# VisionLearningGroup/UDA_PoseEstimation

Hardware: AMD Instinct MI355X
Metric: images/sec (student+teacher step) 256x256 b=32 (higher is better)
Workload: dtype bf16

## Files before the change

### uda_poseestimation_amd/csrc/conv_plan.h

```cpp
#pragma once
#include <atomic>
#include <mutex>
#include <vector>
#include "igemm.h"

struct Policy : udapose_policy {
    Policy() : udapose_policy{} {
        igemm_tile = -1; igemm_h3 = 1; igemm_lean = 1; igemm_short_lds = 1; igemm_tap0 = 1;
        wgrad_tile = -1; wgrad_ksplit = -1; wgrad_fastgeo = 2;
        wgrad_group = 1; wgrad_stages = 128; wgrad_group_stem = 1;
        bn_bwd_fused = 1; bn_fwd_chunked = 1; bn_bwd_chunked = 1; bn_bwd_pre_legacy = 0;
        igemm_wg_min = 512; wgrad_row3 = 1; bn3_mask = 1; stem_fused = 1; debug_sync = 0;
        igemm_big_min = 0; patch_conv = 2; eval_fold = 1; bn_xcd_rows = 1; wgrad_det = 1; igemm_ns3_k = 0;
        timeline = nullptr; wgrad_order = 1; wgrad_fastgeo_strided = 1;
    }
};
inline const Policy& default_policy() { static const Policy p; return p; }

template <auto Kernel>
inline void max_dynamic_lds(int bytes) {
    static std::atomic<unsigned long long> done{0};
    static std::mutex mu;
    int dev = 0;
    (void)hipGetDevice(&dev);
    const unsigned long long bit = 1ull << (dev & 63);
    if (done.load(std::memory_order_acquire) & bit) return;
    std::lock_guard<std::mutex> lk(mu);
    if (done.load(std::memory_order_relaxed) & bit) return;
    (void)hipFuncSetAttribute((const void*)Kernel, hipFuncAttributeMaxDynamicSharedMemorySize, bytes);
    done.fetch_or(bit, std::memory_order_release);
}

struct ConvGeom {
    int N, Hi, Wi, Ci;
    int Co, KH, KW, stride, pad;
    int transposed;
    int reflect;
    int upsample;
    const Policy* pol = nullptr;
    const Policy& policy() const { return pol ? *pol : default_policy(); }
    int Ho() const { return transposed ? (Hi - 1) * stride - 2 * pad + KH : (((Hi << upsample) + 2 * pad - KH) / stride + 1); }
    int Wo() const { return transposed ? (Wi - 1) * stride - 2 * pad + KW : (((Wi << upsample) + 2 * pad - KW) / stride + 1); }
    bool smallc() const { return Ci == 8; }
    int KWp() const { return smallc() ? ((KW + 7) & ~7) : KW; }
    int wtaps() const { return KH * KWp(); }
};

struct TapPlan {
    std::vector<IgTap> taps;
    int nclass = 1;
    IgClass cls[4];
    const IgTap* d_taps = nullptr;
};

const TapPlan* get_tap_plan(const ConvGeom& g, int direction, hipStream_t stream = nullptr);
int conv_prepare(const ConvGeom& g);

int igemm_pick_tile(int M, int Co, int nclass, int K, int h3_ok, const Policy& pol);
int conv_h3_ok(const ConvGeom& g);
int igemm_stat_rows(int M, int Co, int nclass, int tile);
int igemm_launch(IgParams& p, int tile, hipStream_t stream, const Policy& pol);
int wgrad_pick_tile(int Rdim, int Cdim, int smallc, const Policy& pol);
int wgrad_launch(WgParams& p, int tile, int accumulate, hipStream_t stream, const Policy& pol);
// ... 43 lines not shown
```

### uda_poseestimation_amd/csrc/igemm.h

```cpp
#pragma once
#include "common.h"

struct IgTap { int dy, dx, widx, cls; };
struct IgClass { int tap_off, ntaps, oa, ob; };

#define IG_FLAG_REFLECT 1
#define IG_FLAG_UPSAMPLE 2
#define IG_FLAG_RELU 4
#define IG_FLAG_OUT_F32 8
#define IG_FLAG_F32 128
#define IG_FLAG_SPLIT 64
#define IG_FLAG_MIRROR 2048
#define IG_FLAG_TAP0 1024
#define IG_FLAG_BSMASK 32
#define IG_FLAG_SMALLC 16

struct IgParams {
    const elem_t* x;
    const elem_t* w;
    void* y;
    const elem_t* res;
    const float* bias;
    const float* scale;
    float* stats;
    const IgTap* taps;
    int N, Hi, Wi, Ci;
    int Ho, Wo, Co;
    int Hg, Wg;
    int s, os;
    int M;
    int wtaps;
    int flags;
    int nclass;
    IgClass cls[4];
    FastDiv div_hw, div_w;
    int m_tiles, n_tiles;
    int tap0;
    unsigned long long* dbg;
    const elem_t* bs_y;
    const elem_t* bs_z;
    const float* bs_mean;
    const float* bs_invstd;
    const float* bs_gamma;
    const float* bs_beta;
};

struct WgParams {
    const elem_t* dy;
    const elem_t* x;
    float* dw;
    const IgTap* taps;
    int N, Hi, Wi, Ci;
    int Ho, Wo, Co;
    int Hg, Wg;
    int s, os;
    int M;
    int wtaps;
    int flags;
    int nclass;
    IgClass cls[4];
    FastDiv div_hw, div_w;
    int ksplit;
    int msteps_per_split;
    int r_tiles, c_tiles;
    int total_taps;
    int rows_valid;
    int kw;
    unsigned part_stride;
};
struct WgGroupBlk { int prob, local; };
#define WG_FLAG_SWAP 32
#define WG_FLAG_DW_WS 256
#define WG_FLAG_FASTGEO 512
#define WG_FLAG_FAST2 16384
#define WG_FLAG_FASTGEO_S 32768
#define WG_FLAG_ROW3_OK 8192
#define WG_FLAG_ROW3 4096
#define WG_FLAG_ATOMIC 64
```

### uda_poseestimation_amd/csrc/net.hip

```cpp
#include <algorithm>
#include <deque>
#include <functional>
#include <queue>
#include <cstdio>
#include <cstdlib>
#include <string>
#include <type_traits>
#include <vector>
#include "net.h"
#include "pointwise.h"
#include "optim.h"

namespace {

inline size_t align_up(size_t v, size_t a = 256) { return (v + a - 1) / a * a; }
static thread_local int t_dbg_sync = 0;
struct DbgSyncScope { int prev; explicit DbgSyncScope(int on) : prev(t_dbg_sync) { t_dbg_sync = on; } ~DbgSyncScope() { t_dbg_sync = prev; } };
#define CK(expr) do { int _e = (expr); \
    if (t_dbg_sync) { fprintf(stderr, "[udapose] net.hip:%d %s\n", __LINE__, #expr); fflush(stderr); \
        if (hipDeviceSynchronize() != hipSuccess) { fprintf(stderr, "[udapose] FAILED at net.hip:%d\n", __LINE__); return UDAPOSE_ERR_LAUNCH; } } \
    if (_e != UDAPOSE_OK) return _e; } while (0)

struct ConvL {
    ConvGeom g;
// ... 31 lines not shown
    DevTable& operator=(DevTable&& o) noexcept { if (this != &o) { reset(); d = o.d; n = o.n; o.d = nullptr; o.n = 0; } return *this; }
    ~DevTable() { reset(); }
    void reset() { if (d) (void)hipFree(d); d = nullptr; n = 0; }
    int upload(const std::vector<T>& v) {
        reset();
        if (hipMalloc((void**)&d, v.size() * sizeof(T)) != hipSuccess) { d = nullptr; return UDAPOSE_ERR_LAUNCH; }
        if (hipMemcpy(d, v.data(), v.size() * sizeof(T), hipMemcpyHostToDevice) != hipSuccess) { reset(); return UDAPOSE_ERR_LAUNCH; }
        n = v.size();
        return UDAPOSE_OK;
    }
};
template <class J> struct JobTab {
    DevTable<J> jobs; DevTable<int> blk_job, blk_sub;
    int nblocks() const { return (int)blk_job.n; }
    void reset() { jobs.reset(); blk_job.reset(); blk_sub.reset(); }
    int upload(const std::vector<J>& j, const std::vector<int>& bj, const std::vector<int>& bs) {
        if (jobs.upload(j) == UDAPOSE_OK && blk_job.upload(bj) == UDAPOSE_OK && blk_sub.upload(bs) == UDAPOSE_OK) return UDAPOSE_OK;
        reset();
        return UDAPOSE_ERR_LAUNCH;
    }
};
struct PackJobH { const float* src; elem_t* dst; int A, T, B, kind; long long n; };

struct Net {
    int layers[4], K, N, H, W;
    int split_dz_idx = -1;
    Policy policy;
    int f32 = 0;
    int strict = 0;
    int fwd_only = 0;
    struct Scratch { size_t need[6] = {0, 0, 0, 0, 0, 0}, off[6] = {0, 0, 0, 0, 0, 0}; bool sizing = false; } sc;
    int deconv_bias = 0;
    size_t es = 2;
    int n_params = 0, n_buffers = 0;
    std::vector<long long> param_numel;
    ConvL stem; BnL stem_bn;
    size_t x8_off = 0, pool_off = 0, poolidx_off = 0;
    size_t fx8_off = 0, fpool_off = 0;
    int Hs = 0, Ws = 0, Hp = 0, Wp = 0;
    std::vector<Block> blocks;
    ConvL up[3]; BnL up_bn[3];
    ConvL head;
    size_t head_out_off = 0;
    int fc_w_idx = -1, fc_b_idx = -1;
    size_t act_bytes = 0, wpack_bytes = 0, ws_bytes = 0;
    size_t ws_slab = 0, ws_slabf = 0, ws_coef = 0, ws_gbuf[6] = {0, 0, 0, 0, 0, 0}, ws_dyhead = 0, ws_dwtmp = 0, ws_headbwd = 0;
    size_t ws_wgpart = 0, ws_wgpart_bytes = 0;
    size_t gbuf_bytes = 0;
    int Hout = 0, Wout = 0;
    struct PackTab : JobTab<PackJobH> { const void* key0 = nullptr; const void* key1 = nullptr; const void* keyw = nullptr; };
    PackTab pack_fwd, pack_all;
    struct WgGroup {
        float k_beta = -1.f; int k_stages = 0; int k_part = 0;
        bool k_det = false, k_stem = false; int k_order = 0, k_geo_s = 0;
        size_t part_bytes = 0;
        std::vector<std::pair<int, ptrdiff_t>> rel;
        std::vector<size_t> rel_bytes;
        std::vector<int> rel_cls;
        DevTable<WgParams> d_tab[WG_CLASSES]; DevTable<WgGroupBlk> d_blk[WG_CLASSES]; int per_xcd[WG_CLASSES] = {};
        double flops[WG_CLASSES] = {};
        std::vector<std::pair<ptrdiff_t, size_t>> zero;
        DevTable<ZeroJob> d_zero;
        DevTable<SumJob> d_sum; DevTable<int> d_sum_blk; int n_sum_blk = 0;
        int n_sum_ws_blk = 0;
        std::vector<SumJob> h_sum;
        unsigned long long last_use = 0;
    };
    std::deque<WgGroup> wg_groups;
    struct UpdTab : JobTab<TailJob> {
                    const void* k_ps = nullptr; const void* k_pt = nullptr; const void* k_g = nullptr; const void* k_m = nullptr;
                    const void* k_ws = nullptr; const void* k_wt = nullptr;
                    int kind = 0, ngroups = 1; };
    UpdTab upd;
    struct Deferred { const WgGroup* G = nullptr; char* wsA = nullptr; char* wsB = nullptr; char* gA = nullptr; char* gB = nullptr; } deferred;
    const WgGroup* upd_sum_group = nullptr;
    DevTable<BnRunJob> d_runjobs; const void* runjobs_key = nullptr;
    unsigned long long wg_tick = 0;
};

template <class F, class... A> int walk_rc(F& fn, A&... a) {
    if constexpr (std::is_void_v<decltype(fn(a...))>) { fn(a...); return UDAPOSE_OK; }
    else return fn(a...);
}
template <class N, class F> int for_each_layer(N& n, F fn) {
    int rc = walk_rc(fn, n.stem, n.stem_bn);
    for (size_t i = 0; rc == UDAPOSE_OK && i < n.blocks.size(); ++i) {
        auto& b = n.blocks[i];
        if ((rc = walk_rc(fn, b.c1, b.b1)) == UDAPOSE_OK && (rc = walk_rc(fn, b.c2, b.b2)) == UDAPOSE_OK && (rc = walk_rc(fn, b.c3, b.b3)) == UDAPOSE_OK && b.has_ds)
            rc = walk_rc(fn, b.cd, b.bd);
    }
    for (int i = 0; rc == UDAPOSE_OK && i < 3; ++i) rc = walk_rc(fn, n.up[i], n.up_bn[i]);
    return rc;
}
template <class N, class F> int for_each_conv(N& n, F fn) { return for_each_layer(n, [&](auto& c, auto&) { return walk_rc(fn, c); }); }
template <class N, class F> int for_each_bn(N& n, F fn) { return for_each_layer(n, [&](auto&, auto& b) { return walk_rc(fn, b); }); }

size_t act_alloc(Net& n, size_t bytes) { size_t o = n.act_bytes; n.act_bytes = align_up(o + bytes); return o; }
size_t wp_alloc(Net& n, size_t bytes) { size_t o = n.wpack_bytes; n.wpack_bytes = align_up(o + bytes); return o; }

enum { SC_Y = 0, SC_A, SC_B, SC_MID, SC_MID2, SC_DS, SC_COUNT };
size_t sc_take(Net& n, int slot, size_t bytes) {
    if (n.sc.sizing) { n.sc.need[slot] = std::max(n.sc.need[slot], align_up(bytes)); return 0; }
    return n.sc.off[slot];
}
void add_conv(Net& n, ConvL& c, int Hi, int Wi, int Ci, int Co, int K, int stride, int pad, int transposed, size_t in_off, size_t fin_off, bool need_bwd_pack,
              int y_slot = -1) {
    c.g = ConvGeom{n.N, Hi, Wi, Ci, Co, K, K, stride, pad, transposed, 0, 0};
// ... 382 lines not shown
    }
    if (c.g.smallc() && grouped_wgrad && n.policy.wgrad_group_stem) {
    } else if (c.g.smallc()) {
        float* tmp = (float*)(ws + n.ws_dwtmp);
        CK(conv_wgrad(s, c.g, dy, xin, tmp, 0, -1));
        CK(pw_unpack_strided(s, tmp, (float*)grads[c.w_idx], c.g.Co, c.g.KH, c.g.KWp(), c.g.KW, 8, 3, (long)c.g.KH * c.g.KW * 3, (long)c.g.KW * 3, 3, 1,
                             beta));
    } else if (!grouped_wgrad) {
        CK(conv_wgrad(s, c.g, dy, xin, (float*)grads[c.w_idx], beta != 0.f, -1));
    }
    if (need_dx) {
        elem_t* dx = pool.get();
        if (!dx) return UDAPOSE_ERR_ARG;
        CK(conv_dgrad(s, c.g, dy, (const elem_t*)(wpack + c.wb_off), dx, dx_res, dx_f32, next));
        *dx_out = dx;
    }
    return UDAPOSE_OK;
}

DgradBnStat bn_stat_of(const Net& n, const ConvL& c, const BnL& b, const void* const* params, char* act, char* ws, int relu) {
    DgradBnStat st;
    const float* save = (const float*)(act + b.save_off);
    st.y = (const elem_t*)(act + c.y_off);
    st.z = relu == 1 ? (const elem_t*)(act + b.z_off) : nullptr;
    st.mask = (relu == 1 && b.mask_off && n.policy.bn3_mask) ? (const unsigned char*)(act + b.mask_off) : nullptr;
    st.mean = save; st.invstd = save + b.C;
    st.gamma = (const float*)params[b.g_idx]; st.beta = (const float*)params[b.b_idx];
    st.slab = (float*)(ws + n.ws_slabf);
    return st;
}


inline int split_block(const Net& n) { return n.layers[0] + n.layers[1]; }

struct PartSel { bool head_up; int hi, lo; bool stem; };
PartSel part_sel(const Net& n, int part) {
    const int nb = (int)n.blocks.size(), split = split_block(n);
    if (part == 1) return PartSel{true, nb - 1, split, false};
    if (part == 2) return PartSel{false, split - 1, 0, true};
    return PartSel{true, nb - 1, 0, true};
}
template <class N, class F> int for_each_conv_wgrad(N& n, const PartSel& sel, F fn) {
    int rc = UDAPOSE_OK;
    for (int i = 2; sel.head_up && rc == UDAPOSE_OK && i >= 0; --i) rc = walk_rc(fn, n.up[i]);
    for (int bi = sel.hi; rc == UDAPOSE_OK && bi >= sel.lo; --bi) {
        auto& b = n.blocks[bi];
        if ((rc = walk_rc(fn, b.c3)) == UDAPOSE_OK && (rc = walk_rc(fn, b.c2)) == UDAPOSE_OK && (!b.has_ds || (rc = walk_rc(fn, b.cd)) == UDAPOSE_OK))
            rc = walk_rc(fn, b.c1);
    }
    return rc;
}

#define WG_DEAL_RUN 32
struct WgUnit { int prob, base, nblk, st; long load; };
double wg_model_finish(const std::vector<WgUnit>& runs, const std::vector<int>& lst, int slots = 128) {
    std::priority_queue<double, std::vector<double>, std::greater<double>> free_at;
    for (int i = 0; i < slots; ++i) free_at.push(0.0);
    double end = 0.0;
    for (int ui : lst)
        for (int l = 0; l < runs[ui].nblk; ++l) {
            const double t = free_at.top() + runs[ui].st + 4;
            free_at.pop();
            free_at.push(t);
            end = std::max(end, t);
        }
    return end;
}
void wg_deal(const std::vector<WgUnit>& units, int order, std::vector<WgUnit>& runs, std::vector<int> lst[8]) {
    runs.clear();
    for (const WgUnit& u : units) {
        const int step = order == 0 ? u.nblk : WG_DEAL_RUN;
        for (int l0 = 0; l0 < u.nblk; l0 += step) {
            const int cnt = std::min(step, u.nblk - l0);
            runs.push_back(WgUnit{u.prob, u.base + l0, cnt, u.st, (long)cnt * (u.st + 4)});
        }
    }
    std::vector<int> idx(runs.size());
    for (size_t i = 0; i < idx.size(); ++i) idx[i] = (int)i;
    if (order == 0) std::stable_sort(idx.begin(), idx.end(), [&](int a, int b) { return runs[a].load > runs[b].load; });
    else std::stable_sort(idx.begin(), idx.end(), [&](int a, int b) { return runs[a].st != runs[b].st ? runs[a].st > runs[b].st : runs[a].load > runs[b].load; });
    long load[8] = {0, 0, 0, 0, 0, 0, 0, 0};
    for (int k = 0; k < 8; ++k) lst[k].clear();
    for (int ui : idx) {
        int x = 0;
        for (int k = 1; k < 8; ++k) if (load[k] < load[x]) x = k;
        load[x] += runs[ui].load;
        lst[x].push_back(ui);
    }
}

int build_wg_group(Net& n, Net::WgGroup& G, void* const* grads, float beta, int part, bool sizing = false, size_t* need = nullptr) {
    const PartSel sel = part_sel(n, part);
    const bool upper = sel.head_up, lower = sel.stem;
    std::vector<WgParams> tab[WG_CLASSES];
    std::vector<WgUnit> units[WG_CLASSES];
    G.zero.clear();
    G.rel.clear();
    G.rel_bytes.clear();
    G.rel_cls.clear();
    for (int t = 0; t < WG_CLASSES; ++t) G.flops[t] = 0.0;
    std::vector<SumJob> sums;
    size_t part_cur = 0;
    const bool det = n.policy.wgrad_det && n.policy.wgrad_group;
    auto make_partial = [&](WgParams& p, long long dst_off, int dst_ws, int Cdim) -> int {
        const int ms_total = (p.M + 63) / 64, per = (ms_total + p.ksplit - 1) / p.ksplit;
        const int ks_eff = (ms_total + per - 1) / per;
        const size_t span = (size_t)p.rows_valid * p.wtaps * Cdim;
        if (span >= (1ull << 31) || (span & 3)) return UDAPOSE_ERR_UNSUPPORTED;
        p.flags = (p.flags & ~WG_FLAG_ATOMIC) | WG_FLAG_DW_WS;
        p.dw = (float*)(n.ws_wgpart + part_cur);
        p.part_stride = (unsigned)span;
        sums.push_back(SumJob{(long long)(n.ws_wgpart + part_cur), dst_off, (unsigned)span, (unsigned)span, ks_eff, dst_ws, dst_ws ? 0.f : beta, 0});
        part_cur = align_up(part_cur + (size_t)ks_eff * span * sizeof(float));
        return UDAPOSE_OK;
    };
    auto emit = [&](int t, const WgParams& p, double fl) {
        const int prob = (int)tab[t].size();
        tab[t].push_back(p);
        G.flops[t] += fl;
        const int nblk = p.r_tiles * p.c_tiles * p.total_taps;
        const int ms_total = (p.M + 63) / 64, per = (ms_total + p.ksplit - 1) / p.ksplit;
        for (int z = 0; z < p.ksplit; ++z) {
            const int st = std::min(per, ms_total - z * per);
            if (st > 0) units[t].push_back(WgUnit{prob, z * nblk, nblk, st, (long)nblk * (st + 4)});
        }
    };
    auto add_geom = [&](const ConvGeom& g, int w_idx, size_t dy_off, size_t in_off, int rows_valid) -> int {
        if (g.smallc()) return UDAPOSE_OK;
        WgParams p;
        double fl = 0.0;
        const ptrdiff_t drel = sizing ? 0 : (const char*)grads[w_idx] - (const char*)grads[0];
        G.rel.push_back({w_idx, drel});
        CK(conv_wgrad_params(g, (const elem_t*)dy_off, (const elem_t*)in_off, (float*)drel, rows_valid, &p, &fl));
        const int t = wgrad_group_plan(p, beta != 0.f, n.policy.wgrad_stages, n.policy);
        if (t < 0) return UDAPOSE_ERR_UNSUPPORTED;
        G.rel_bytes.push_back((size_t)p.rows_valid * p.wtaps * ((p.flags & WG_FLAG_SWAP) ? p.Co : p.Ci) * sizeof(float));
        if (p.ksplit > 1) {
            const bool swap = (p.flags & WG_FLAG_SWAP) != 0;
            if (det) CK(make_partial(p, (long long)drel, 0, swap ? p.Co : p.Ci));
            else if (beta == 0.f) G.zero.push_back({drel, (size_t)p.rows_valid * p.wtaps * (swap ? p.Co : p.Ci) * sizeof(float)});
        }
        G.rel_cls.push_back(t);
        emit(t, p, fl);
        return UDAPOSE_OK;
    };
    if (upper) {
        ConvGeom hg = n.head.g;
        hg.Co = 64;
        CK(add_geom(hg, n.head.w_idx, n.ws_dyhead, n.head.in_off, n.K));
        G.flops[1] -= 2.0 * n.N * n.Hout * n.Wout * 256.0 * (64 - n.K);
    }
    if (lower && n.policy.wgrad_group_stem) {
        WgParams p;
        double fl = 0.0;
        CK(conv_wgrad_params(n.stem.g, (const elem_t*)n.stem.dy_off, (const elem_t*)n.stem.in_off, (float*)n.ws_dwtmp, -2, &p, &fl));
        p.flags |= WG_FLAG_DW_WS;
        const int t = wgrad_group_plan(p, 1, n.policy.wgrad_stages, n.policy);
        if (t != 1) return UDAPOSE_ERR_UNSUPPORTED;
        if (det) CK(make_partial(p, (long long)n.ws_dwtmp, 1, 64));
        emit(t, p, fl);
    }
    CK(for_each_conv_wgrad(n, sel, [&](const ConvL& c) { return add_geom(c.g, c.w_idx, c.dy_off, c.in_off, -1); }));
    if (sizing) { if (need) *need = part_cur; return UDAPOSE_OK; }
    if (part_cur > n.ws_wgpart_bytes) return UDAPOSE_ERR_NOT_PREPARED;
    for (int t = 0; t < WG_CLASSES; ++t) {
        G.d_tab[t].reset();
        G.d_blk[t].reset();
        G.per_xcd[t] = 0;
        if (tab[t].empty()) continue;
        std::vector<int> deal[8];
        std::vector<WgUnit> runs;
        wg_deal(units[t], n.policy.wgrad_order, runs, deal);
        std::vector<WgGroupBlk> lst[8];
        for (int x = 0; x < 8; ++x)
            for (int ui : deal[x]) {
                const WgUnit& u = runs[ui];
                for (int l = 0; l < u.nblk; ++l) lst[x].push_back(WgGroupBlk{u.prob, u.base + l});
            }
        size_t per = 0;
        for (int k = 0; k < 8; ++k) per = std::max(per, lst[k].size());
        std::vector<WgGroupBlk> flat(8 * per, WgGroupBlk{-1, 0});
        for (int k = 0; k < 8; ++k) std::copy(lst[k].begin(), lst[k].end(), flat.begin() + k * per);
        CK(G.d_tab[t].upload(tab[t]));
        CK(G.d_blk[t].upload(flat));
        G.per_xcd[t] = (int)per;
    }
    G.d_zero.reset();
    bool granular = !G.zero.empty();
    for (auto& z : G.zero) granular = granular && (z.second % 16 == 0) && ((((size_t)(const char*)grads[0]) + (size_t)z.first) % 16 == 0);
    if (granular) {
        std::vector<ZeroJob> zj;
        for (auto& z : G.zero) zj.push_back(ZeroJob{(long long)z.first, (long long)(z.second / 16)});
        CK(G.d_zero.upload(zj));
    }
    G.d_sum.reset();
    G.d_sum_blk.reset();
    G.n_sum_blk = 0; G.n_sum_ws_blk = 0;
    if (!sums.empty()) {
        std::vector<int> blk;
        for (const int ws_jobs : {0, 1})
            for (size_t j = 0; j < sums.size(); ++j) {
                if ((sums[j].dst_ws != 0) != (ws_jobs != 0)) continue;
                for (unsigned c = 0; c < (sums[j].n + UDAPOSE_SPLIT_SUM_CHUNK - 1u) / UDAPOSE_SPLIT_SUM_CHUNK; ++c) {
                    blk.push_back((int)j); blk.push_back((int)c);
                    G.n_sum_ws_blk += ws_jobs;
                }
            }
        CK(G.d_sum.upload(sums));
        CK(G.d_sum_blk.upload(blk));
        G.n_sum_blk = (int)(blk.size() / 2);
    }
    G.h_sum = sums;
    G.k_beta = beta; G.k_stages = n.policy.wgrad_stages; G.k_part = part;
    G.k_det = det; G.k_stem = n.policy.wgrad_group_stem != 0; G.part_bytes = part_cur; G.k_order = n.policy.wgrad_order; G.k_geo_s = n.policy.wgrad_fastgeo_strided;
    return UDAPOSE_OK;
}

size_t wg_partial_bytes(Net& n) {
    Net::WgGroup G;
    size_t need = 0;
    if (build_wg_group(n, G, nullptr, 0.f, 0, true, &need) != UDAPOSE_OK) return 0;
    return need;
}

Net::WgGroup* find_wg_group(Net& n, void* const* grads, float beta, int part) {
    const bool det = n.policy.wgrad_det && n.policy.wgrad_group, stem = n.policy.wgrad_group_stem != 0;
    for (auto& g : n.wg_groups) {
        if (g.k_beta != beta || g.k_stages != n.policy.wgrad_stages || g.k_part != part || g.k_det != det || g.k_stem != stem ||
            g.k_order != n.policy.wgrad_order || g.k_geo_s != n.policy.wgrad_fastgeo_strided) continue;
        if (g.k_det && g.part_bytes > n.ws_wgpart_bytes) continue;
        bool same = true;
        for (auto& r : g.rel)
            if ((const char*)grads[r.first] - (const char*)grads[0] != r.second) { same = false; break; }
        if (same) return &g;
    }
    return nullptr;
}
int bind_wg_groups(Net& n, void* const* grads) {
    for (const int part : {0, 1, 2})
        for (const float beta : {0.f, 1.f}) {
            if (find_wg_group(n, grads, beta, part)) continue;
            n.wg_groups.emplace_back();
            Net::WgGroup* G = &n.wg_groups.back();
            const int rc = build_wg_group(n, *G, grads, beta, part);
            if (rc != UDAPOSE_OK) { n.wg_groups.pop_back(); return rc; }
            G->last_use = ++n.wg_tick;
        }
    return UDAPOSE_OK;
}
int wg_before(hipStream_t s, Net& n, Net::WgGroup* G, char* ws, void* const* grads, bool with_stem) {
    G->last_use = ++n.wg_tick;
    if (G->d_zero.d) {
        CK(pw_zero_multi(s, G->d_zero.d, (int)G->d_zero.n, grads[0]));
    } else {
        for (auto& z : G->zero)
            if (pw_zero(s, (char*)grads[0] + z.first, z.second) != UDAPOSE_OK) return UDAPOSE_ERR_LAUNCH;
    }
    const ConvGeom& sg = n.stem.g;
    if (with_stem && !G->k_det && pw_zero(s, ws + n.ws_dwtmp, (size_t)sg.Co * sg.KH * 8 * 8 * sizeof(float)) != UDAPOSE_OK) return UDAPOSE_ERR_LAUNCH;
    return UDAPOSE_OK;
}
int wg_after(hipStream_t s, Net& n, Net::WgGroup* G, char* ws, void* const* grads, float beta, bool with_stem, bool sums_done = false) {
    if (G->n_sum_blk && !sums_done) CK(pw_split_sum(s, G->d_sum.d, G->d_sum_blk.d, G->n_sum_blk, ws, (char*)grads[0]));
    const ConvGeom& sg = n.stem.g;
    if (with_stem)
        CK(pw_unpack_strided(s, (const float*)(ws + n.ws_dwtmp), (float*)grads[n.stem.w_idx], sg.Co, sg.KH, sg.KWp(), sg.KW, 8, 3,
                             (long)sg.KH * sg.KW * 3, (long)sg.KW * 3, 3, 1, beta));
    return UDAPOSE_OK;
}
bool wg_overlap(const Net& n, const Net::WgGroup* GA, void* const* gradsA, const Net::WgGroup* GB, void* const* gradsB, bool with_stem) {
    auto span = [&](const Net::WgGroup* G, void* const* grads, uintptr_t& lo, uintptr_t& hi) {
        lo = UINTPTR_MAX; hi = 0;
        auto add = [&](int idx, size_t bytes) {
            const uintptr_t a = (uintptr_t)grads[idx];
            lo = std::min(lo, a); hi = std::max(hi, a + bytes);
        };
        for (size_t i = 0; i < G->rel.size(); ++i) add(G->rel[i].first, G->rel_bytes[i]);
        if (with_stem) add(n.stem.w_idx, (size_t)n.stem.g.Co * n.stem.g.KH * n.stem.g.KW * 3 * sizeof(float));
    };
// ... 377 lines not shown
```

### uda_poseestimation_amd/csrc/wgrad.hip

```cpp
#include <stdlib.h>
#include "conv_plan.h"
#include "mma_tile.h"
#include "pointwise.h"

namespace {

template <int RT, int CT, int WR, int WC>
struct WgCfg {
    static constexpr int TR = RT / WR, TC = CT / WC;
    static constexpr int MT = TR / 16, NT = TC / 16;
    static constexpr int PSTR = RT * 2 + 32, QSTR = CT * 2 + 32;
    static constexpr int P_BYTES = 32 * PSTR, Q_BYTES = 32 * QSTR;
    static constexpr int P_CH = (32 * RT / 8 + 255) / 256, Q_CH = (32 * CT / 8 + 255) / 256;
    static constexpr int LDS_BYTES = 2 * (P_BYTES + Q_BYTES);
};

template <int MT, int NT>
__device__ __forceinline__ void wg_store_tile(const f32x4 (&acc)[MT][NT], int lane, int row0, int col0, int Rdim, int rows_valid, int Cdim, int wtaps, int widx,
                                              float* dw, size_t part_off, bool atomic) {
#pragma unroll
    for (int i = 0; i < MT; ++i)
#pragma unroll
        for (int j = 0; j < NT; ++j)
#pragma unroll
// ... 559 lines not shown
        }

    for (int st = 0; st < nsteps; ++st) {
        const int buf = st % NS;
        ring.step(st, nsteps, issue_stage);
        const char* P = smem + buf * R::STAGE1;
        const char* Q = P + R::P_BYTES;
#pragma unroll
        for (int kk = 0; kk < 2; ++kk) {
            union F8 { struct { s16x4 a, b; } s; elem8 v; u32x4 w; };
            F8 af[2];
#pragma unroll
            for (int i = 0; i < 2; ++i) {
                const int col = wr * 32 + i * 16 + 4 * pp;
#pragma unroll
                for (int h = 0; h < 2; ++h) {
                    const int row = 32 * kk + 16 * h + 4 * g + qq;
                    const int off = wfrag_off<64>(row, col);
                    const s16x4 v = __builtin_amdgcn_ds_read_tr16_b64_v4i16(LDS_PTR(s16x4, P + off));
                    if (h == 0) af[i].s.a = v; else af[i].s.b = v;
                }
            }
#pragma unroll
            for (int t = 0; t < 3; ++t) {
                F8 bfr[2];
#pragma unroll
                for (int j = 0; j < 2; ++j) {
                    const int col = wc * 32 + j * 16 + 4 * pp;
#pragma unroll
                    for (int h = 0; h < 2; ++h) {
                        const int row = 32 * kk + 16 * h + 4 * g + qq + t;
                        const int off = wfrag_off<64>(row, col);
                        const s16x4 v = __builtin_amdgcn_ds_read_tr16_b64_v4i16(LDS_PTR(s16x4, Q + off));
                        if (h == 0) bfr[j].s.a = v; else bfr[j].s.b = v;
                    }
                }
#pragma unroll
                for (int i = 0; i < 2; ++i) {
                    F8 a = af[i];
                    if (t == 0) { a.w[0] &= mL[kk][0]; a.w[1] &= mL[kk][1]; a.w[2] &= mL[kk][2]; a.w[3] &= mL[kk][3]; }
                    if (t == 2) { a.w[0] &= mR[kk][0]; a.w[1] &= mR[kk][1]; a.w[2] &= mR[kk][2]; a.w[3] &= mR[kk][3]; }
#pragma unroll
                    for (int j = 0; j < 2; ++j) acc[t][i][j] = UDAPOSE_MFMA_16x16x32(a.v, bfr[j].v, acc[t][i][j]);
                }
            }
        }
    }

#pragma unroll
    for (int t = 0; t < 3; ++t)
        wg_store_tile(acc[t], lane, r0 + wr * 32, c0 + wc * 32, p.Co, p.rows_valid, p.Ci, p.wtaps, 3 * by + t, p.dw, part_off, (p.flags & WG_FLAG_ATOMIC) != 0);
}

template <int RT, int CT, int WR, int WC, int NS, int PX>
__device__ __forceinline__ void wgrad_run_body(const WgParams& p, const uint32_t bx, const uint32_t by, const uint32_t bz, char* smem,
                                               const uintptr_t x_base, const uintptr_t dy_base, const uintptr_t dw_base) {
    if constexpr (RT == 64 && CT == 64 && PX == 64) {
        if (p.flags & WG_FLAG_ROW3) { wgrad_row3_body<NS>(p, bx, by, bz, smem, x_base, dy_base, dw_base); return; }
    }
    if (p.flags & WG_FLAG_FAST2) wgrad_fast2_body<RT, CT, WR, WC, NS, PX>(p, bx, by, bz, smem, x_base, dy_base, dw_base);
    else if (p.flags & WG_FLAG_FASTGEO) wgrad_dma_body<RT, CT, WR, WC, NS, PX, 1>(p, bx, by, bz, smem, x_base, dy_base, dw_base);
    else if (p.flags & WG_FLAG_FASTGEO_S) wgrad_dma_body<RT, CT, WR, WC, NS, PX, 2>(p, bx, by, bz, smem, x_base, dy_base, dw_base);
    else wgrad_dma_body<RT, CT, WR, WC, NS, PX>(p, bx, by, bz, smem, x_base, dy_base, dw_base);
}

template <int RT, int CT, int WR, int WC, int NS>
__global__ __launch_bounds__(256) void wgrad_dma_kernel(const WgParams p) {
    extern __shared__ __attribute__((aligned(16))) char smem[];
    const uint32_t gxy = gridDim.x * gridDim.y;
    const uint32_t lin = xcd_remap(blockIdx.x + gridDim.x * (blockIdx.y + gridDim.y * blockIdx.z), gxy * gridDim.z);
    const uint32_t bz = lin / gxy, bxy = lin - bz * gxy;
    const uint32_t by = bxy / gridDim.x, bx = bxy - by * gridDim.x;
    wgrad_run_body<RT, CT, WR, WC, NS, 64>(p, bx, by, bz, smem, 0, 0, 0);
}

template <int RT, int CT, int WR, int WC, int NS, int PX>
__device__ __forceinline__ void wgrad_group_dispatch(const WgParams* __restrict__ tab, const WgGroupBlk* __restrict__ blk, const uint32_t per_xcd,
                                                     const char* x_base, const char* dy_base, char* dw_base, const WgParams* __restrict__ tab2,
                                                     const WgGroupBlk* __restrict__ blk2, const char* x_base2, const char* dy_base2, char* dw_base2,
                                                     char* smem) {
    uint32_t slot = blockIdx.x >> 3;
    if (tab2) {
        if (slot & 1u) { tab = tab2; blk = blk2; x_base = x_base2; dy_base = dy_base2; dw_base = dw_base2; }
        slot >>= 1;
    }
    const WgGroupBlk b = blk[(blockIdx.x & 7u) * per_xcd + slot];
    if (b.prob < 0) return;
    const WgParams& p = tab[b.prob];
    const uint32_t gx = (uint32_t)(p.r_tiles * p.c_tiles), gxy = gx * (uint32_t)p.total_taps;
    const uint32_t bz = (uint32_t)b.local / gxy, bxy = (uint32_t)b.local - bz * gxy;
    const uint32_t by = bxy / gx, bx = bxy - by * gx;
    wgrad_run_body<RT, CT, WR, WC, NS, PX>(p, bx, by, bz, smem, (uintptr_t)x_base, (uintptr_t)dy_base, (uintptr_t)dw_base);
}

template <int RT, int CT, int WR, int WC, int NS, int PX, bool STAMP = false>
__global__ __launch_bounds__(256) __attribute__((amdgpu_waves_per_eu(4))) void wgrad_dma_group_kernel(const WgParams* __restrict__ tab, const WgGroupBlk* __restrict__ blk,
                                                              const uint32_t per_xcd, const char* x_base, const char* dy_base, char* dw_base,
                                                              const WgParams* __restrict__ tab2, const WgGroupBlk* __restrict__ blk2,
                                                              const char* x_base2, const char* dy_base2, char* dw_base2,
                                                              unsigned long long* __restrict__ stamps) {
    extern __shared__ __attribute__((aligned(16))) char smem[];
    if constexpr (STAMP) {
        unsigned long long* const st = stamps + (size_t)blockIdx.x * 8;
        const unsigned long long t0 = __builtin_amdgcn_s_memrealtime();
        uint32_t slot = blockIdx.x >> 3, pass = 0;
        if (tab2) { pass = slot & 1u; slot >>= 1; }
        const WgGroupBlk b = (pass ? blk2 : blk)[(blockIdx.x & 7u) * per_xcd + slot];
        long long stages = 0;
        if (b.prob >= 0) {
            const WgParams& p = (pass ? tab2 : tab)[b.prob];
            const uint32_t gxy = (uint32_t)(p.r_tiles * p.c_tiles) * (uint32_t)p.total_taps;
            const int bz = (int)((uint32_t)b.local / gxy), ms_total = (p.M + 63) / 64;
            stages = ms_total - bz * p.msteps_per_split < p.msteps_per_split ? ms_total - bz * p.msteps_per_split : p.msteps_per_split;
            if (p.flags & WG_FLAG_ROW3) stages |= 1ll << 32;
            if (p.flags & IG_FLAG_SMALLC) stages |= 1ll << 33;
            if (p.flags & WG_FLAG_FASTGEO_S) stages |= 1ll << 34;
            if (p.flags & WG_FLAG_SWAP) stages |= 1ll << 35;
            if (p.s == 2) stages |= 1ll << 36;
        }
        wgrad_group_dispatch<RT, CT, WR, WC, NS, PX>(tab, blk, per_xcd, x_base, dy_base, dw_base, tab2, blk2, x_base2, dy_base2, dw_base2, smem);
        __syncthreads();
        if (threadIdx.x == 0) {
            st[0] = t0; st[1] = __builtin_amdgcn_s_memrealtime(); st[2] = blockIdx.x & 7u; st[3] = slot;
            st[4] = (unsigned long long)(long long)b.prob; st[5] = (unsigned long long)stages; st[6] = pass; st[7] = RT;
        }
    } else {
        wgrad_group_dispatch<RT, CT, WR, WC, NS, PX>(tab, blk, per_xcd, x_base, dy_base, dw_base, tab2, blk2, x_base2, dy_base2, dw_base2, smem);
    }
}

template <int RT, int CT, int WR, int WC, int NS, int PX, bool STAMP = false>
int launch_wd_group(const WgParams* d_tab, const WgGroupBlk* d_blk, int per_xcd, const void* x_base, const void* dy_base, void* dw_base,
                    hipStream_t stream, const WgParams* d_tab2 = nullptr, const WgGroupBlk* d_blk2 = nullptr, const void* x_base2 = nullptr,
                    const void* dy_base2 = nullptr, void* dw_base2 = nullptr, unsigned long long* stamps = nullptr) {
    using C = WdCfg<RT, CT, WR, WC, NS, PX>;
    constexpr int LDS = (RT == 64 && CT == 64 && PX == 64 && Row3Cfg::lds_bytes(NS) > C::LDS_BYTES) ? Row3Cfg::lds_bytes(NS) : C::LDS_BYTES;
    max_dynamic_lds<wgrad_dma_group_kernel<RT, CT, WR, WC, NS, PX, STAMP>>(LDS);
    hipLaunchKernelGGL((wgrad_dma_group_kernel<RT, CT, WR, WC, NS, PX, STAMP>), dim3(8 * per_xcd * (d_tab2 ? 2 : 1)), dim3(256), LDS, stream, d_tab, d_blk,
                       (uint32_t)per_xcd, (const char*)x_base, (const char*)dy_base, (char*)dw_base, d_tab2, d_blk2, (const char*)x_base2,
                       (const char*)dy_base2, (char*)dw_base2, stamps);
    return udapose_check_launch();
}

template <int RT, int CT, int WR, int WC, int NS>
int launch_wd(WgParams& p, hipStream_t stream) {
    using C = WdCfg<RT, CT, WR, WC, NS>;
    constexpr int LDS = (RT == 64 && CT == 64 && Row3Cfg::lds_bytes(NS) > C::LDS_BYTES) ? Row3Cfg::lds_bytes(NS) : C::LDS_BYTES;
    const bool swap = (p.flags & WG_FLAG_SWAP) != 0;
    const int Rdim = swap ? p.Ci : p.Co, Cdim = swap ? p.Co : p.Ci;
    p.r_tiles = (Rdim + RT - 1) / RT;
    p.c_tiles = (Cdim + CT - 1) / CT;
    max_dynamic_lds<wgrad_dma_kernel<RT, CT, WR, WC, NS>>(LDS);
    dim3 grid(p.r_tiles * p.c_tiles, p.total_taps, p.ksplit);
    hipLaunchKernelGGL((wgrad_dma_kernel<RT, CT, WR, WC, NS>), grid, dim3(256), LDS, stream, p);
    return udapose_check_launch();
}

template <int RT, int CT, int WR, int WC>
int launch_wg(WgParams& p, hipStream_t stream) {
    using C = WgCfg<RT, CT, WR, WC>;
    const bool swap = (p.flags & WG_FLAG_SWAP) != 0;
    const bool smallc = (p.flags & IG_FLAG_SMALLC) != 0;
    const int Rdim = swap ? p.Ci : p.Co, Cdim = swap ? p.Co : p.Ci;
    p.r_tiles = (Rdim + RT - 1) / RT;
    p.c_tiles = smallc ? 1 : (Cdim + CT - 1) / CT;
    const int tapsy = smallc ? p.total_taps / 4 : p.total_taps;
    dim3 grid(p.r_tiles * p.c_tiles, tapsy, p.ksplit);
    hipLaunchKernelGGL((wgrad_kernel<RT, CT, WR, WC>), grid, dim3(256), C::LDS_BYTES, stream, p);
    return udapose_check_launch();
}

}

static bool wg_fastgeo_ok(const WgParams& p, const Policy& pol) {
    const bool pow2 = ((p.Hi & (p.Hi - 1)) | (p.Wi & (p.Wi - 1))) == 0;
    return pol.wgrad_fastgeo && !(p.flags & (IG_FLAG_SMALLC | WG_FLAG_SWAP)) && p.s == 1 && p.os == 1 && p.nclass == 1 && p.Hg == p.Hi && p.Wg == p.Wi &&
           p.Hg == p.Ho && p.Wg == p.Wo && pow2 && p.Hi > 0 && p.M < (1 << 24) && p.Ci < (1 << 24) && p.Co < (1 << 24) &&
           (long long)p.M * (p.Ci > p.Co ? p.Ci : p.Co) < (1ll << 31);
}

static bool wg_fastgeo_strided_ok(const WgParams& p, const Policy& pol) {
    if (!pol.wgrad_fastgeo || !pol.wgrad_fastgeo_strided || wg_fastgeo_ok(p, pol)) return false;
    const int dims[6] = {p.Hg, p.Wg, p.Hi, p.Wi, p.Ho, p.Wo};
    for (int d : dims) if (d <= 0 || (d & (d - 1))) return false;
    if ((p.s != 1 && p.s != 2) || (p.os != 1 && p.os != 2) || p.Ho != p.Hg * p.os || p.Wo != p.Wg * p.os) return false;
    if (p.nclass < 1 || p.nclass > 4) return false;
    for (int c = 0; c < p.nclass; ++c)
        if (p.cls[c].oa < 0 || p.cls[c].oa >= p.os || p.cls[c].ob < 0 || p.cls[c].ob >= p.os) return false;
    if (p.flags & IG_FLAG_SMALLC) {
// ... 45 lines not shown
        p.flags |= WG_FLAG_ROW3;
        p.total_taps = 3;
    }
    const long tiles = (long)((Rdim + RT[tile] - 1) / RT[tile]) * (smallc ? 1 : (Cdim + CT[tile] - 1) / CT[tile]) *
                       (smallc ? p.total_taps / 4 : p.total_taps);
    const bool dma = !smallc && (tile == 0 || tile == 1) && (p.Ci % 64 == 0) && (p.Co % 64 == 0);
    const int ms_total = dma ? (p.M + 63) / 64 : (p.M + 31) / 32;
    int ks = wg_split_count(tiles, ms_total, tile, 1 << 30);
    if (pol.wgrad_ksplit > 0) { ks = pol.wgrad_ksplit; while (ks > 1 && ms_total / ks < 1) ks /= 2; }
    p.ksplit = ks;
    p.part_stride = 0;
    p.msteps_per_split = (ms_total + ks - 1) / ks;
    if (ks > 1 || accumulate) p.flags |= WG_FLAG_ATOMIC; else p.flags &= ~WG_FLAG_ATOMIC;
    if (ks > 1 && !accumulate) {
        const size_t n = (size_t)Rdim * p.wtaps * Cdim;
        if (pw_zero(stream, p.dw, n * sizeof(float)) != UDAPOSE_OK) return UDAPOSE_ERR_LAUNCH;
    }
    wg_classify(p, pol, dma);
    if (dma) return tile == 0 ? launch_wd<128, 128, 2, 2, 2>(p, stream) : launch_wd<64, 64, 2, 2, 4>(p, stream);
    switch (tile) {
        case 0: return launch_wg<128, 128, 2, 2>(p, stream);
        case 1: return launch_wg<64, 64, 2, 2>(p, stream);
        case 2: return launch_wg<64, 32, 2, 2>(p, stream);
        case 3: return launch_wg<32, 128, 1, 4>(p, stream);
        default: return UDAPOSE_ERR_ARG;
    }
}

int wgrad_group_plan(WgParams& p, int accumulate, int stages_per_block, const Policy& pol) {
    const bool smallc = (p.flags & IG_FLAG_SMALLC) != 0;
    const bool swap = (p.flags & WG_FLAG_SWAP) != 0;
    if (smallc && (swap || p.Co % 64 != 0 || p.kw <= 0 || p.kw > 8)) return -1;
    if (!smallc && (p.Ci % 64 != 0 || p.Co % 64 != 0)) return -1;
    const int Rdim = swap ? p.Ci : p.Co, Cdim = smallc ? 64 : (swap ? p.Co : p.Ci);
    p.div_hw = make_fastdiv((uint32_t)(p.Hg * p.Wg));
    p.div_w = make_fastdiv((uint32_t)p.Wg);
    int tile = (Rdim >= 128 && Cdim >= 128) ? 0 : 1;
    if (wg_row3_ok(p, pol)) {
        tile = 1;
        p.flags |= WG_FLAG_ROW3;
        p.total_taps = 3;
    }
    const int TRr = tile == 0 ? 128 : 64, TCc = tile == 1 ? 64 : 128;
    p.r_tiles = (Rdim + TRr - 1) / TRr;
    p.c_tiles = (Cdim + TCc - 1) / TCc;
    const int ms_total = (p.M + 63) / 64;
    int ks = (ms_total + stages_per_block / 2) / stages_per_block;
    if (ks < 1) ks = 1;
    p.ksplit = ks;
    p.part_stride = 0;
    p.msteps_per_split = (ms_total + ks - 1) / ks;
    if (ks > 1 || accumulate) p.flags |= WG_FLAG_ATOMIC; else p.flags &= ~WG_FLAG_ATOMIC;
    wg_classify(p, pol, true);
    return tile;
}

int wgrad_group_launch(hipStream_t stream, int tile, const WgParams* d_tab, const WgGroupBlk* d_blk, int per_xcd, const void* x_base,
                       const void* dy_base, void* dw_base, const WgParams* d_tab2, const WgGroupBlk* d_blk2, const void* x_base2,
                       const void* dy_base2, void* dw_base2, unsigned long long* stamps) {
    if (per_xcd <= 0) return UDAPOSE_OK;
    if (stamps) {
        if (tile == 0) return launch_wd_group<128, 128, 2, 2, 2, 32, true>(d_tab, d_blk, per_xcd, x_base, dy_base, dw_base, stream, d_tab2, d_blk2, x_base2, dy_base2, dw_base2, stamps);
        return launch_wd_group<64, 64, 2, 2, 2, 64, true>(d_tab, d_blk, per_xcd, x_base, dy_base, dw_base, stream, d_tab2, d_blk2, x_base2, dy_base2, dw_base2, stamps);
    }
    if (tile == 0) return launch_wd_group<128, 128, 2, 2, 2, 32>(d_tab, d_blk, per_xcd, x_base, dy_base, dw_base, stream, d_tab2, d_blk2, x_base2, dy_base2, dw_base2);
    return launch_wd_group<64, 64, 2, 2, 2, 64>(d_tab, d_blk, per_xcd, x_base, dy_base, dw_base, stream, d_tab2, d_blk2, x_base2, dy_base2, dw_base2);
}

int wgrad_parts_plan(int M, int Ci, int Co, int total_taps, int* tile_out) {
    const int tile = (Co >= 128 && Ci >= 128 && total_taps >= 9) ? 0 : 1;
    const int RT = tile == 0 ? 128 : 64;
    const long tiles = (long)((Co + RT - 1) / RT) * ((Ci + RT - 1) / RT) * total_taps;
    const int ms_total = (M + 63) / 64;
    const int ks = wg_split_count(tiles, ms_total, tile, 64);
    if (tile_out) *tile_out = tile;
    return ks;
}

int wgrad_launch_parts(WgParams& p, float* parts, hipStream_t stream) {
    if (p.Ci % 64 || p.Co % 64 || (p.flags & (IG_FLAG_SMALLC | WG_FLAG_SWAP | WG_FLAG_ROW3_OK))) return UDAPOSE_ERR_ARG;
    int tile = 1;
    const int ks = wgrad_parts_plan(p.M, p.Ci, p.Co, p.total_taps, &tile);
    p.div_hw = make_fastdiv((uint32_t)(p.Hg * p.Wg));
    p.div_w = make_fastdiv((uint32_t)p.Wg);
    p.ksplit = ks;
    p.msteps_per_split = ((p.M + 63) / 64 + ks - 1) / ks;
    p.dw = parts;
    p.part_stride = (unsigned)((size_t)p.Co * p.wtaps * p.Ci);
    p.flags &= ~(WG_FLAG_ATOMIC | WG_FLAG_FASTGEO | WG_FLAG_FAST2 | WG_FLAG_FASTGEO_S | WG_FLAG_ROW3);
    return tile == 0 ? launch_wd<128, 128, 2, 2, 2>(p, stream) : launch_wd<64, 64, 2, 2, 4>(p, stream);
}
```

Baseline: 2034.

## Add stem row-group wgrad path sharing dy tile across kernel rows

Adds a specialized weight-gradient body for the small-channel stem conv that processes up to three kernel rows per block. One dy tile staged in LDS is reused against several x row tiles, which cuts redundant dy loads and block count. The scheduler cost model is adjusted for the heavier per-stage work, and the policy default enables the path. The new path carries more accumulators, which adds register pressure, and each group now does more serialized work.

```diff
diff --git a/uda_poseestimation_amd/csrc/conv_plan.h b/uda_poseestimation_amd/csrc/conv_plan.h
--- a/uda_poseestimation_amd/csrc/conv_plan.h
+++ b/uda_poseestimation_amd/csrc/conv_plan.h
@@ -8,7 +8,7 @@
     Policy() : udapose_policy{} {
         igemm_tile = -1; igemm_h3 = 1; igemm_lean = 1; igemm_short_lds = 1; igemm_tap0 = 1;
         wgrad_tile = -1; wgrad_ksplit = -1; wgrad_fastgeo = 2;
-        wgrad_group = 1; wgrad_stages = 128; wgrad_group_stem = 1;
+        wgrad_group = 1; wgrad_stages = 128; wgrad_group_stem = 2;
         bn_bwd_fused = 1; bn_fwd_chunked = 1; bn_bwd_chunked = 1; bn_bwd_pre_legacy = 0;
         igemm_wg_min = 512; wgrad_row3 = 1; bn3_mask = 1; stem_fused = 1; debug_sync = 0;
         igemm_big_min = 0; patch_conv = 2; eval_fold = 1; bn_xcd_rows = 1; wgrad_det = 1; igemm_ns3_k = 0;
diff --git a/uda_poseestimation_amd/csrc/igemm.h b/uda_poseestimation_amd/csrc/igemm.h
--- a/uda_poseestimation_amd/csrc/igemm.h
+++ b/uda_poseestimation_amd/csrc/igemm.h
@@ -76,4 +76,5 @@
 #define WG_FLAG_FASTGEO_S 32768
 #define WG_FLAG_ROW3_OK 8192
 #define WG_FLAG_ROW3 4096
+#define WG_FLAG_STEMROWS 65536
 #define WG_FLAG_ATOMIC 64
diff --git a/uda_poseestimation_amd/csrc/net.hip b/uda_poseestimation_amd/csrc/net.hip
--- a/uda_poseestimation_amd/csrc/net.hip
+++ b/uda_poseestimation_amd/csrc/net.hip
@@ -107,7 +107,7 @@
     PackTab pack_fwd, pack_all;
     struct WgGroup {
         float k_beta = -1.f; int k_stages = 0; int k_part = 0;
-        bool k_det = false, k_stem = false; int k_order = 0, k_geo_s = 0;
+        bool k_det = false; int k_stem = 0, k_order = 0, k_geo_s = 0;
         size_t part_bytes = 0;
         std::vector<std::pair<int, ptrdiff_t>> rel;
         std::vector<size_t> rel_bytes;
@@ -596,6 +596,7 @@
 }
 
 #define WG_DEAL_RUN 32
+#define WG_STEMROWS_STAGE_W 5
 struct WgUnit { int prob, base, nblk, st; long load; };
 double wg_model_finish(const std::vector<WgUnit>& runs, const std::vector<int>& lst, int slots = 128) {
     std::priority_queue<double, std::vector<double>, std::greater<double>> free_at;
@@ -665,8 +666,10 @@
         const int nblk = p.r_tiles * p.c_tiles * p.total_taps;
         const int ms_total = (p.M + 63) / 64, per = (ms_total + p.ksplit - 1) / p.ksplit;
         for (int z = 0; z < p.ksplit; ++z) {
-            const int st = std::min(per, ms_total - z * per);
-            if (st > 0) units[t].push_back(WgUnit{prob, z * nblk, nblk, st, (long)nblk * (st + 4)});
+            int st = std::min(per, ms_total - z * per);
+            if (st <= 0) continue;
+            if (p.flags & WG_FLAG_STEMROWS) st = (st * WG_STEMROWS_STAGE_W + 3) / 4;
+            units[t].push_back(WgUnit{prob, z * nblk, nblk, st, (long)nblk * (st + 4)});
         }
     };
     auto add_geom = [&](const ConvGeom& g, int w_idx, size_t dy_off, size_t in_off, int rows_valid) -> int {
@@ -756,7 +759,7 @@
     }
     G.h_sum = sums;
     G.k_beta = beta; G.k_stages = n.policy.wgrad_stages; G.k_part = part;
-    G.k_det = det; G.k_stem = n.policy.wgrad_group_stem != 0; G.part_bytes = part_cur; G.k_order = n.policy.wgrad_order; G.k_geo_s = n.policy.wgrad_fastgeo_strided;
+    G.k_det = det; G.k_stem = n.policy.wgrad_group_stem; G.part_bytes = part_cur; G.k_order = n.policy.wgrad_order; G.k_geo_s = n.policy.wgrad_fastgeo_strided;
     return UDAPOSE_OK;
 }
 
@@ -768,7 +771,8 @@
 }
 
 Net::WgGroup* find_wg_group(Net& n, void* const* grads, float beta, int part) {
-    const bool det = n.policy.wgrad_det && n.policy.wgrad_group, stem = n.policy.wgrad_group_stem != 0;
+    const bool det = n.policy.wgrad_det && n.policy.wgrad_group;
+    const int stem = n.policy.wgrad_group_stem;
     for (auto& g : n.wg_groups) {
         if (g.k_beta != beta || g.k_stages != n.policy.wgrad_stages || g.k_part != part || g.k_det != det || g.k_stem != stem ||
             g.k_order != n.policy.wgrad_order || g.k_geo_s != n.policy.wgrad_fastgeo_strided) continue;
diff --git a/uda_poseestimation_amd/csrc/wgrad.hip b/uda_poseestimation_amd/csrc/wgrad.hip
--- a/uda_poseestimation_amd/csrc/wgrad.hip
+++ b/uda_poseestimation_amd/csrc/wgrad.hip
@@ -635,11 +635,121 @@
         wg_store_tile(acc[t], lane, r0 + wr * 32, c0 + wc * 32, p.Co, p.rows_valid, p.Ci, p.wtaps, 3 * by + t, p.dw, part_off, (p.flags & WG_FLAG_ATOMIC) != 0);
 }
 
+struct StemRowsCfg {
+    static constexpr int RMAX = 3, PX = 32, TILE = PX * 128, STAGE1 = (1 + RMAX) * TILE;
+    static constexpr int lds_bytes(int ns) { return ns * STAGE1; }
+    static constexpr int groups(int kh) { return (kh + RMAX - 1) / RMAX; }
+};
+__device__ __forceinline__ int stemrows_first(int g, int kh, int ng) {
+    const int b = kh / ng, r = kh - b * ng;
+    return g * b + (g < r ? g : r);
+}
+template <int NS>
+__device__ __forceinline__ void wgrad_stemrows_body(const WgParams& gp, const uint32_t bx, const uint32_t by, const uint32_t bz, char* smem,
+                                                    const uintptr_t x_base, const uintptr_t dy_base, const uintptr_t dw_base) {
+    using R = StemRowsCfg;
+    static_assert(NS == 2, "a stage's DMA count varies with the group: the ring must wait for all of them (vmcnt 0), as the 2-stage one does");
+    struct {
+        const elem_t* dy; const elem_t* x; float* dw;
+        int Hi, Wi, Ci, Co, Hg, Wg, s, M, wtaps, flags, ksplit, rows_valid, kw;
+    } p = {(const elem_t*)((uintptr_t)gp.dy + dy_base), (const elem_t*)((uintptr_t)gp.x + x_base),
+           (float*)((uintptr_t)gp.dw + ((gp.flags & WG_FLAG_DW_WS) ? dy_base : dw_base)), gp.Hi, gp.Wi, gp.Ci, gp.Co, gp.Hg, gp.Wg, gp.s, gp.M, gp.wtaps,
+           gp.flags, gp.ksplit, gp.rows_valid, gp.kw};
+    const int tid = threadIdx.x, lane = tid & 63, wid = __builtin_amdgcn_readfirstlane(tid >> 6);
+    const int wr = wid >> 1, wc = wid & 1;
+    const int r0 = (int)bx * 64;
+    const int row_a = stemrows_first((int)by, p.wtaps, gp.total_taps);
+    const int nr = __builtin_amdgcn_readfirstlane(stemrows_first((int)by + 1, p.wtaps, gp.total_taps) - row_a);
+    const IgTap tp0 = gp.taps[row_a];
+    struct { int dy, dx, widx; } tp = {__builtin_amdgcn_readfirstlane(tp0.dy), __builtin_amdgcn_readfirstlane(tp0.dx),
+                                       __builtin_amdgcn_readfirstlane(tp0.widx)};
+    const WgSplit split = wg_split<64>(p.M, p.ksplit, bz, gp.part_stride);
+    const int mb0 = split.ms0 * 64, nsub = split.nsteps * 2;
+    const size_t part_off = split.part_off;
+    const char* zsrc = (const char*)g_wzero16;
+    const auto lg2 = [](int v) { return 31 - __builtin_clz((unsigned)(v > 0 ? v : 1)); };
+    const int lgw = lg2(p.Wi), lg_hwi = lgw + lg2(p.Hi), lg_wg = lg2(p.Wg), lg_hwg = lg_wg + lg2(p.Hg), lgs = p.s >> 1;
+    const int lrow = lane >> 3, pch = lane & 7;
+
+    auto issue_stage = [&](int st, int buf) __attribute__((always_inline)) {
+        char* S = smem + buf * R::STAGE1 + wid * 1024;
+        const int row = wid * 8 + lrow;
+        const int lc = pch ^ wswz<64>(row);
+        const unsigned m = (unsigned)(mb0 + st * R::PX + row);
+        const bool okm = m < (unsigned)p.M;
+        const unsigned n = m >> lg_hwg, ii = (m >> lg_wg) & (unsigned)(p.Hg - 1), jj = m & (unsigned)(p.Wg - 1);
+        const int dch = r0 + lc * 8;
+        const unsigned od = __umul24(m, (unsigned)p.Co) + (unsigned)dch;
+        lds_dma16((okm && dch < p.Co) ? (const char*)p.dy + (size_t)od * 2 : zsrc, S);
+        const unsigned wl = (jj << lgs) + (unsigned)tp.dx + (unsigned)lc;
+        const bool okc = okm && wl < (unsigned)p.Wi && lc < p.kw;
+        const unsigned xcol = (n << lg_hwi) + wl;
+#pragma unroll
+        for (int r = 0; r < R::RMAX; ++r) {
+            if (r < nr) {
+                const unsigned hi = (ii << lgs) + (unsigned)(tp.dy + r);
+                const unsigned ox = __umul24(xcol + (hi << lgw), (unsigned)p.Ci);
+                lds_dma16((okc && hi < (unsigned)p.Hi) ? (const char*)p.x + (size_t)ox * 2 : zsrc, S + (1 + r) * R::TILE);
+            }
+        }
+    };
+
+    f32x4 acc[R::RMAX][2][2];
+#pragma unroll
+    for (int r = 0; r < R::RMAX; ++r)
+#pragma unroll
+        for (int i = 0; i < 2; ++i)
+#pragma unroll
+            for (int j = 0; j < 2; ++j) acc[r][i][j] = (f32x4){0.f, 0.f, 0.f, 0.f};
+
+    Ring<NS, 1 + R::RMAX> ring;
+    ring.prologue(nsub, issue_stage);
+
+    const int g = lane >> 4, li = lane & 15, qq = li >> 2, pp = li & 3;
+    int a_lo[2][2], b_lo[2][2];
+#pragma unroll
+    for (int h = 0; h < 2; ++h)
+#pragma unroll
+        for (int i = 0; i < 2; ++i) {
+            a_lo[i][h] = wfrag_off<64>(16 * h + 4 * g + qq, wr * 32 + i * 16 + 4 * pp);
+            b_lo[i][h] = wfrag_off<64>(16 * h + 4 * g + qq, wc * 32 + i * 16 + 4 * pp);
+        }
+
+    for (int st = 0; st < nsub; ++st) {
+        ring.step(st, nsub, issue_stage);
+        const char* S = smem + (st % NS) * R::STAGE1;
+        elem8 af[2];
+#pragma unroll
+        for (int i = 0; i < 2; ++i) af[i] = tr_frag(S + a_lo[i][0], S + a_lo[i][1]);
+#pragma unroll
+        for (int r = 0; r < R::RMAX; ++r) {
+            if (r < nr) {
+                const char* Q = S + (1 + r) * R::TILE;
+                elem8 bfr[2];
+#pragma unroll
+                for (int j = 0; j < 2; ++j) bfr[j] = tr_frag(Q + b_lo[j][0], Q + b_lo[j][1]);
+#pragma unroll
+                for (int i = 0; i < 2; ++i)
+#pragma unroll
+                    for (int j = 0; j < 2; ++j) acc[r][i][j] = UDAPOSE_MFMA_16x16x32(af[i], bfr[j], acc[r][i][j]);
+            }
+        }
+    }
+
+#pragma unroll
+    for (int r = 0; r < R::RMAX; ++r)
+        if (r < nr)
+            wg_store_tile(acc[r], lane, r0 + wr * 32, wc * 32, p.Co, p.rows_valid, 64, p.wtaps, tp.widx + r, p.dw, part_off, (p.flags & WG_FLAG_ATOMIC) != 0);
+}
+
 template <int RT, int CT, int WR, int WC, int NS, int PX>
 __device__ __forceinline__ void wgrad_run_body(const WgParams& p, const uint32_t bx, const uint32_t by, const uint32_t bz, char* smem,
                                                const uintptr_t x_base, const uintptr_t dy_base, const uintptr_t dw_base) {
     if constexpr (RT == 64 && CT == 64 && PX == 64) {
         if (p.flags & WG_FLAG_ROW3) { wgrad_row3_body<NS>(p, bx, by, bz, smem, x_base, dy_base, dw_base); return; }
+    }
+    if constexpr (RT == 64 && CT == 64 && PX == 64 && NS == 2) {
+        if (p.flags & WG_FLAG_STEMROWS) { wgrad_stemrows_body<NS>(p, bx, by, bz, smem, x_base, dy_base, dw_base); return; }
     }
     if (p.flags & WG_FLAG_FAST2) wgrad_fast2_body<RT, CT, WR, WC, NS, PX>(p, bx, by, bz, smem, x_base, dy_base, dw_base);
     else if (p.flags & WG_FLAG_FASTGEO) wgrad_dma_body<RT, CT, WR, WC, NS, PX, 1>(p, bx, by, bz, smem, x_base, dy_base, dw_base);
@@ -700,6 +810,7 @@
             if (p.flags & WG_FLAG_FASTGEO_S) stages |= 1ll << 34;
             if (p.flags & WG_FLAG_SWAP) stages |= 1ll << 35;
             if (p.s == 2) stages |= 1ll << 36;
+            if (p.flags & WG_FLAG_STEMROWS) stages |= 1ll << 37;
         }
         wgrad_group_dispatch<RT, CT, WR, WC, NS, PX>(tab, blk, per_xcd, x_base, dy_base, dw_base, tab2, blk2, x_base2, dy_base2, dw_base2, smem);
         __syncthreads();
@@ -718,6 +829,7 @@
                     const void* dy_base2 = nullptr, void* dw_base2 = nullptr, unsigned long long* stamps = nullptr) {
     using C = WdCfg<RT, CT, WR, WC, NS, PX>;
     constexpr int LDS = (RT == 64 && CT == 64 && PX == 64 && Row3Cfg::lds_bytes(NS) > C::LDS_BYTES) ? Row3Cfg::lds_bytes(NS) : C::LDS_BYTES;
+    static_assert(!(RT == 64 && CT == 64 && PX == 64 && NS == 2) || StemRowsCfg::lds_bytes(NS) <= LDS, "the row-group form's ring fits the class's allocation");
     max_dynamic_lds<wgrad_dma_group_kernel<RT, CT, WR, WC, NS, PX, STAMP>>(LDS);
     hipLaunchKernelGGL((wgrad_dma_group_kernel<RT, CT, WR, WC, NS, PX, STAMP>), dim3(8 * per_xcd * (d_tab2 ? 2 : 1)), dim3(256), LDS, stream, d_tab, d_blk,
                        (uint32_t)per_xcd, (const char*)x_base, (const char*)dy_base, (char*)dw_base, d_tab2, d_blk2, (const char*)x_base2,
@@ -869,6 +981,12 @@
     p.msteps_per_split = (ms_total + ks - 1) / ks;
     if (ks > 1 || accumulate) p.flags |= WG_FLAG_ATOMIC; else p.flags &= ~WG_FLAG_ATOMIC;
     wg_classify(p, pol, true);
+    p.flags &= ~WG_FLAG_STEMROWS;
+    if (smallc && pol.wgrad_group_stem >= 2 && (p.flags & WG_FLAG_FASTGEO_S) && tile == 1 && p.c_tiles == 1 && p.os == 1 && p.nclass == 1 &&
+        p.cls[0].oa == 0 && p.cls[0].ob == 0 && p.Hg == p.Ho && p.Wg == p.Wo && p.total_taps == p.wtaps && p.wtaps >= 2) {
+        p.flags |= WG_FLAG_STEMROWS;
+        p.total_taps = StemRowsCfg::groups(p.wtaps);
+    }
     return tile;
 }
 
```

After: 2034. About the same (-0.0%).
